# DoHoonKim8/stark-verifier

Measured on AMD Instinct MI355X. Metric: recursive plonky2 proofs/sec (Semaphore d=20), higher is better.
Workload: dtype u64 (Goldilocks field, integer); 1 GPU; recursive: per unit one Semaphore signal (group 2^20, n=2^13, blowup 8, 28 FRI queries, 16 PoW bits, zk) + the recursive proof verifying it (n=2^14, same FRI parameters); 128 units per GPU per step, 10 prover contexts per GPU; all_gather of (nullifier|topic) + Poseidon aggregation root per step; parallelism=independent proofs sharded over ranks, no data-path collective, exchange=none (one rank): gl355_aggregation_root over the local leaves, units_proven_in_process=1674

## Files before the change

include/gl355.h:

```cpp
#ifndef GL355_H
#define GL355_H
#include <stddef.h>
#include <stdint.h>

#ifdef __cplusplus
extern "C" {
#endif

#define GL355_OK 0
#define GL355_E_INVALID_ARG (-1)
#define GL355_E_NO_DEVICE (-2)
#define GL355_E_OOM (-3)
#define GL355_E_HIP (-4)
#define GL355_E_UNSUPPORTED (-5)
#define GL355_E_WITNESS (-6)
#define GL355_E_VERIFY (-7)

#define GL355_P UINT64_C(0xFFFFFFFF00000001)
#define GL355_COSET_SHIFT UINT64_C(7)
#define GL355_SALT_SIZE 4
#define GL355_MAX_UNITS 16

typedef struct gl355_ctx gl355_ctx;
typedef struct gl355_oracle gl355_oracle;
// ... 122 lines not shown
int32_t gl355_quotient_values(gl355_ctx* ctx, const gl355_circuit* circuit, const gl355_oracle* constants_sigmas,
                              const gl355_oracle* wires, const gl355_oracle* zs_partial_products, const uint64_t* k_is,
                              const uint64_t* betas, const uint64_t* gammas, const uint64_t* alphas,
                              const uint64_t pi_hash[4], uint64_t* values);

typedef struct { const gl355_oracle* oracle; uint32_t column; } gl355_poly_ref;
int32_t gl355_deep_batch(gl355_ctx* ctx, const gl355_poly_ref* polys, uint32_t n_polys,
                         const uint64_t alpha[2], const uint64_t z[2], uint64_t* acc);
int32_t gl355_eval_polys(gl355_ctx* ctx, const gl355_poly_ref* polys, uint32_t n_polys,
                         const uint64_t z[2], uint64_t* out);
int32_t gl355_lde_ext(gl355_ctx* ctx, const uint64_t* coeffs, uint32_t log_n, uint32_t rate_bits,
                      uint64_t shift, uint64_t* out);

int32_t gl355_fri_fold(gl355_ctx* ctx, const uint64_t* coeffs, uint64_t n, const uint64_t beta[2], uint64_t* out);
int32_t gl355_fri_layer_commit_h(gl355_ctx* ctx, int32_t hasher, const uint64_t* values, uint64_t n, uint32_t cap_height,
                                 uint64_t* leaves, uint64_t* digests, uint64_t* cap);
int32_t gl355_fri_layer_commit(gl355_ctx* ctx, const uint64_t* values, uint64_t n, uint32_t cap_height,
                               uint64_t* leaves, uint64_t* digests, uint64_t* cap);

int32_t gl355_pow_grind_h(gl355_ctx* ctx, int32_t hasher, const uint64_t state[12], uint32_t pos, uint32_t bits, uint64_t start,
                          uint64_t* witness);
int32_t gl355_pow_grind(gl355_ctx* ctx, const uint64_t state[12], uint32_t pos, uint32_t bits,
                        uint64_t start, uint64_t* witness);

typedef struct {
    uint64_t state[12];
    uint64_t in_buf[8];
    uint32_t in_len;
    uint64_t out_buf[8];
    uint32_t out_len;
    int32_t hasher;
} gl355_challenger;
int32_t gl355_challenger_init(gl355_challenger* c);
int32_t gl355_challenger_init_h(gl355_challenger* c, int32_t hasher);
int32_t gl355_challenger_observe(gl355_challenger* c, const uint64_t* elems, uint64_t n);
int32_t gl355_challenger_squeeze(gl355_challenger* c, uint64_t* out, uint64_t n);
int32_t gl355_challenger_pow_state(const gl355_challenger* c, uint64_t state[12], uint32_t* pos);
int32_t gl355_host_poseidon_permute(uint64_t state[12]);
int32_t gl355_host_hash_no_pad(const uint64_t* in, uint64_t len, uint64_t out[4]);
int32_t gl355_host_permute_h(int32_t hasher, uint64_t state[12]);
int32_t gl355_host_hash_no_pad_h(int32_t hasher, const uint64_t* in, uint64_t len, uint64_t out[4]);
int32_t gl355_poseidon_gate_witness(const uint64_t inputs[12], uint64_t swap, uint64_t wires[135]);

int32_t gl355_fri_prove(gl355_ctx* ctx, const uint64_t* final_coeffs, uint32_t log_n, uint32_t rate_bits,
                        uint32_t cap_height, const uint32_t* arity_bits, uint32_t n_layers, uint32_t pow_bits,
                        uint32_t num_queries, gl355_challenger* ch, uint64_t* caps, uint64_t* final_poly,
// ... 166 lines not shown
```

stark-verifier_amd/_lib.py:

```python
import ctypes as C
import os

_HERE = os.path.dirname(os.path.abspath(__file__))
LIB_PATH = os.path.join(_HERE, "lib", "libgl355.so")

u64p = C.POINTER(C.c_uint64)
vp = C.c_void_p


class Gl355Error(RuntimeError):
    def __init__(self, code, msg):
        super().__init__("gl355 error %d: %s" % (code, msg))
        self.code = code


class PolyRef(C.Structure):
    _fields_ = [("oracle", vp), ("column", C.c_uint32)]


class Challenger(C.Structure):
    _fields_ = [("state", C.c_uint64 * 12), ("in_buf", C.c_uint64 * 8), ("in_len", C.c_uint32),
                ("out_buf", C.c_uint64 * 8), ("out_len", C.c_uint32), ("hasher", C.c_int32)]


# ... 123 lines not shown
    "gl355_witness_replay_segmented": (C.c_int32, [vp, C.c_uint64, C.c_uint64, vp, C.c_uint32, C.c_uint32, vp, C.c_uint64, vp, C.c_uint64, C.c_uint32,
                                                   C.POINTER(C.c_uint64)]),
    "gl355_witness_replay": (C.c_int32, [vp, C.c_uint64, vp, C.c_uint64, vp, C.c_uint64, C.c_uint32, C.POINTER(C.c_uint64)]),
    "gl355_quotient": (C.c_int32, [vp, C.POINTER(Circuit), vp, vp, vp, vp, vp, vp, vp, vp, vp]),
    "gl355_quotient_values": (C.c_int32, [vp, C.POINTER(Circuit), vp, vp, vp, vp, vp, vp, vp, vp, vp]),
    "gl355_challenger_init": (C.c_int32, [C.POINTER(Challenger)]),
    "gl355_challenger_init_h": (C.c_int32, [C.POINTER(Challenger), C.c_int32]),
    "gl355_challenger_observe": (C.c_int32, [C.POINTER(Challenger), vp, C.c_uint64]),
    "gl355_challenger_squeeze": (C.c_int32, [C.POINTER(Challenger), vp, C.c_uint64]),
    "gl355_challenger_pow_state": (C.c_int32, [C.POINTER(Challenger), vp, C.POINTER(C.c_uint32)]),
    "gl355_host_poseidon_permute": (C.c_int32, [vp]),
    "gl355_host_hash_no_pad": (C.c_int32, [vp, C.c_uint64, vp]),
    "gl355_host_hash_no_pad_h": (C.c_int32, [C.c_int32, vp, C.c_uint64, vp]),
    "gl355_host_permute_h": (C.c_int32, [C.c_int32, vp]),
    "gl355_poseidon_gate_witness": (C.c_int32, [vp, C.c_uint64, vp]),
    "gl355_deep_batch": (C.c_int32, [vp, C.POINTER(PolyRef), C.c_uint32, vp, vp, vp]),
    "gl355_eval_polys": (C.c_int32, [vp, C.POINTER(PolyRef), C.c_uint32, vp, vp]),
    "gl355_lde_ext": (C.c_int32, [vp, vp, C.c_uint32, C.c_uint32, C.c_uint64, vp]),
    "gl355_fri_fold": (C.c_int32, [vp, vp, C.c_uint64, vp, vp]),
    "gl355_fri_layer_commit_h": (C.c_int32, [vp, C.c_int32, vp, C.c_uint64, C.c_uint32, vp, vp, vp]),
    "gl355_fri_layer_commit": (C.c_int32, [vp, vp, C.c_uint64, C.c_uint32, vp, vp, vp]),
    "gl355_pow_grind_h": (C.c_int32, [vp, C.c_int32, vp, C.c_uint32, C.c_uint32, C.c_uint64, C.POINTER(C.c_uint64)]),
    "gl355_pow_grind": (C.c_int32, [vp, vp, C.c_uint32, C.c_uint32, C.c_uint64, C.POINTER(C.c_uint64)]),
    "gl355_comm_unique_id": (C.c_int32, [C.c_int32, C.c_char_p]),
    "gl355_comm_host_id": (C.c_int32, [C.c_char_p, C.c_uint16, C.c_char_p]),
    "gl355_comm_create": (C.c_int32, [vp, C.c_int32, C.c_char_p, C.c_int32, C.c_int32, C.POINTER(vp)]),
    "gl355_comm_destroy": (C.c_int32, [vp]),
    "gl355_comm_info": (C.c_int32, [vp, C.POINTER(C.c_int32), C.POINTER(C.c_int32), C.POINTER(C.c_int32)]),
    "gl355_comm_last_error": (C.c_char_p, [vp]),
    "gl355_gather_digests": (C.c_int32, [vp, vp, C.c_uint64, vp]),
    "gl355_comm_barrier": (C.c_int32, [vp]),
    "gl355_comm_max_f64": (C.c_int32, [vp, C.POINTER(C.c_double)]),
    "gl355_aggregation_root": (C.c_int32, [vp, vp, C.c_uint64, C.c_uint32, vp]),
    "gl355_bn254_fr_ntt": (C.c_int32, [vp, vp, C.c_uint32, C.c_int32]),
    "gl355_bn254_fr_coset_ntt": (C.c_int32, [vp, vp, C.c_uint32, C.c_uint32, vp, C.c_int32, vp]),
    "gl355_bn254_g1_msm": (C.c_int32, [vp, vp, vp, C.c_uint64, vp]),
    "gl355_bn254_g1_msm_batch": (C.c_int32, [vp, vp, vp, C.c_uint64, C.c_uint32, vp]),
    "gl355_bn254_g1_msm_prepare": (C.c_int32, [vp, vp, C.c_uint64, C.POINTER(vp)]),
    "gl355_bn254_g1_msm_prepared": (C.c_int32, [vp, vp, vp, C.c_uint32, vp]),
    "gl355_bn254_g1_msm_bases_free": (C.c_int32, [vp, vp]),
    "gl355_bn254_g1_fixed_base_mul": (C.c_int32, [vp, vp, vp, C.c_uint64, vp]),
    "gl355_bn254_g1_fft": (C.c_int32, [vp, vp, C.c_uint32, C.c_int32]),
    "gl355_kzg_setup": (C.c_int32, [vp, vp, C.c_uint32, vp, vp]),
    "gl355_kzg_lagrange_from_powers": (C.c_int32, [vp, vp, C.c_uint64, C.c_uint32, vp]),
    "gl355_kzg_commit": (C.c_int32, [vp, vp, vp, C.c_uint32, C.c_int32, vp]),
    "gl355_kzg_open": (C.c_int32, [vp, vp, vp, C.c_uint32, vp, vp, vp, vp]),
# ... 32 lines not shown
```

stark-verifier_amd/api.py:

```python
import ctypes as C

import numpy as np

from . import _lib
from ._lib import Gl355Error, PolyRef

P = (1 << 64) - (1 << 32) + 1
COSET_SHIFT = 7
SALT_SIZE = 4


def _ptr(x):
    if x is None:
        return None
    if isinstance(x, np.ndarray):
        assert x.dtype == np.uint64 and x.flags["C_CONTIGUOUS"], "need C-contiguous uint64"
        return x.ctypes.data_as(C.c_void_p)
    if isinstance(x, int):
        return C.c_void_p(x)
    if hasattr(x, "data_ptr"):
        assert x.is_contiguous()
        return C.c_void_p(x.data_ptr())
    raise TypeError("unsupported buffer type %r" % type(x))

# ... 144 lines not shown

    def fri_fold(self, coeffs_ext, beta):
        c = _u64(coeffs_ext)
        n = c.size // 2
        out = np.empty(n, dtype=np.uint64)
        b = _u64(beta)
        self.check(self.lib.gl355_fri_fold(self.h, _ptr(c), n, _ptr(b), _ptr(out)))
        return out

    def fri_layer_commit(self, values_ext, cap_height):
        v = _u64(values_ext)
        n = v.size // 2
        leaves = np.empty((n // 2, 4), dtype=np.uint64)
        digests = np.empty((2 * (n // 2 - (1 << cap_height)), 4), dtype=np.uint64)
        cap = np.empty((1 << cap_height, 4), dtype=np.uint64)
        self.check(self.lib.gl355_fri_layer_commit(self.h, _ptr(v), n, cap_height, _ptr(leaves), _ptr(digests), _ptr(cap)))
        return MerkleTree._from_parts(self, leaves, digests, cap, cap_height)

    def pow_grind(self, state, pos, bits, start=0):
        s = _u64(state)
        w = C.c_uint64()
        self.check(self.lib.gl355_pow_grind(self.h, _ptr(s), pos, bits, start, C.byref(w)))
        return w.value

    def zs_partial_products(self, wires, sigmas, k_is, max_degree, beta, gamma):
        w, s, k = _u64(wires), _u64(sigmas), _u64(k_is)
        n_routed, n = w.shape
        n_chunks = (n_routed + max_degree - 1) // max_degree
        z = np.empty(n, dtype=np.uint64)
        pp = np.empty((n_chunks - 1, n), dtype=np.uint64)
        self.check(self.lib.gl355_zs_partial_products(self.h, _ptr(w), _ptr(s), _ptr(k), int(n).bit_length() - 1,
                                                      n_routed, max_degree, beta, gamma, _ptr(z), _ptr(pp)))
        return z, pp


class _Hasher:
    ID = HASH_POSEIDON

    def __init__(self, ctx):
        self.ctx = ctx

    def permute(self, states):
        st = _u64(states).copy()
        s2 = st.reshape(-1, 12)
        self.ctx.check(self.ctx.lib.gl355_permute_h(self.ctx.h, self.ID, _ptr(s2), s2.shape[0]))
        return st
# ... 191 lines not shown
```

stark-verifier_amd/csrc/capi.hip:

```cpp
#include "gl355_internal.h"

using namespace gl355;

namespace gl355 {

int32_t ntt_dev(Ctx* ctx, uint64_t* data, uint32_t log_n, uint32_t batch, uint64_t stride, bool inverse,
                uint64_t coset_shift) {
    if (batch == 0) return GL355_OK;
    const uint64_t n = 1ull << log_n;
    if (log_n > 24) return ctx->fail(GL355_E_UNSUPPORTED, "ntt: log_n > 24 unsupported");
    NttPlan p;
    p.in = data; p.out = data; p.in_col_stride = stride; p.out_col_stride = stride;
    p.log_n = log_n; p.batch = batch; p.inverse = inverse;
    const bool coset = coset_shift != 0 && gl_canon(coset_shift) != 1;
    if (!inverse) {
        if (coset) GL355_TRY(ctx->pow_tables(coset_shift, &p.pre_lo, &p.pre_hi));
        p.out_bitrev = false;
        return ntt_run(ctx, p);
    }
    p.scale = gl_canon(gl_inv(n % GL_P));
    if (log_n <= 14) {
        if (coset) GL355_TRY(ctx->pow_tables(gl_inv(coset_shift), &p.post_lo, &p.post_hi));
        return ntt_run(ctx, p);
    }
// ... 503 lines not shown
    if (cap_height > lg) return ctx->fail(GL355_E_INVALID_ARG, "fri_layer_commit: cap_height too large");
    const uint64_t n_cap = 1ull << cap_height, n_dig = 2 * (n_leaves - n_cap);
    Staged sv(ctx), sl(ctx), sd(ctx), sc(ctx);
    GL355_TRY(sv.open(values, n * 16, 1));
    GL355_TRY(sl.open(leaves, n * 16, 2));
    GL355_TRY(sd.open(digests, n_dig * 32, 2));
    GL355_TRY(sc.open(cap, n_cap * 32, 2));
    GL355_TRY(fri_layer_leaves_dev(ctx, sv.as<uint64_t>(), n, sl.as<uint64_t>()));
    GL355_TRY(merkle_build_any(ctx, hasher, sl.as<uint64_t>(), n_leaves, 4, false, 0, cap_height, sd.as<uint64_t>(), sc.as<uint64_t>()));
    GL355_TRY(sl.finish());
    GL355_TRY(sd.finish());
    return sc.finish();
}
int32_t gl355_pow_grind(gl355_ctx* h, const uint64_t state[12], uint32_t pos, uint32_t bits, uint64_t start, uint64_t* witness) {
    return gl355_pow_grind_h(h, GL355_HASH_POSEIDON, state, pos, bits, start, witness);
}
int32_t gl355_pow_grind_h(gl355_ctx* h, int32_t hasher, const uint64_t state[12], uint32_t pos, uint32_t bits, uint64_t start,
                          uint64_t* witness) {
    CTX_OR_FAIL(h);
    HASHER_OR_FAIL(hasher);
    if (!state || !witness || pos >= 8) return ctx->fail(GL355_E_INVALID_ARG, "pow_grind: bad argument");
    return pow_grind_any(ctx, hasher, state, pos, bits, start, witness);
}

int32_t gl355_zs_partial_products(gl355_ctx* h, const uint64_t* wires, const uint64_t* sigmas, const uint64_t* k_is,
                                  uint32_t log_n, uint32_t n_routed, uint32_t max_degree, uint64_t beta, uint64_t gamma,
                                  uint64_t* z_out, uint64_t* pp_out) {
    CTX_OR_FAIL(h);
    if (n_routed == 0 || max_degree == 0 || log_n > 24) return ctx->fail(GL355_E_INVALID_ARG, "zs_partial_products: bad shape");
    const uint64_t n = 1ull << log_n;
    const uint32_t n_chunks = (n_routed + max_degree - 1) / max_degree;
    Staged sw(ctx), ss(ctx), sk(ctx), sz(ctx), sp(ctx);
    GL355_TRY(sw.open(wires, (uint64_t)n_routed * n * 8, 1));
    GL355_TRY(ss.open(sigmas, (uint64_t)n_routed * n * 8, 1));
    GL355_TRY(sk.open(k_is, (uint64_t)n_routed * 8, 1));
    GL355_TRY(sz.open(z_out, n * 8, 2));
    GL355_TRY(sp.open(pp_out, (uint64_t)(n_chunks - 1) * n * 8, 2));
    GL355_TRY(zs_partial_products_dev(ctx, sw.as<uint64_t>(), ss.as<uint64_t>(), sk.as<uint64_t>(), log_n, n_routed, max_degree,
                                      beta, gamma, sz.as<uint64_t>(), sp.as<uint64_t>()));
    GL355_TRY(sz.finish());
    return sp.finish();
}

}
```

stark-verifier_amd/csrc/gl355_internal.h:

```cpp
#pragma once
#include <hip/hip_runtime.h>
#include <stdint.h>
#include <string.h>

#include <algorithm>
#include <map>
#include <mutex>
#include <string>
#include <vector>

#include "../../include/gl355.h"
#include "gl_field.cuh"
#include "merkle_common.cuh"

namespace gl355 { struct Ctx; }

struct gl355_oracle {
    struct gl355::Ctx* ctx;
    uint32_t log_n, rate_bits, batch, leaf_len, cap_height;
    uint64_t* coeffs;
    uint64_t* lde;
    uint64_t* digests;
    uint64_t* cap;
    uint64_t n_digests;
// ... 164 lines not shown
int32_t two_to_one_dev(Ctx* ctx, const uint64_t* l, const uint64_t* r, uint64_t n, uint64_t* out);
int32_t open_batch_dev(Ctx* ctx, const uint64_t* lde, uint64_t stride, uint32_t leaf_len, const uint64_t* digests,
                       uint32_t log_n, uint32_t cap_height, const uint64_t* idx_dev, uint32_t n_idx, uint64_t* leaves_out,
                       uint64_t* sib_out);
int32_t open_batch_ex_dev(Ctx* ctx, const uint64_t* leaves, uint64_t stride, uint32_t leaf_len, const uint64_t* digests,
                          uint32_t log_n, uint32_t cap_height, const uint64_t* idx_dev, uint32_t idx_shift, uint32_t n_idx,
                          uint64_t* leaves_out, uint64_t leaf_out_stride, uint64_t* sib_out, uint64_t sib_out_stride);
void host_bn254_permute(uint64_t state[12]);
int32_t merkle_build_any(Ctx* ctx, int32_t hasher, const uint64_t* leaves, uint64_t n_leaves, uint32_t leaf_len, bool col_major,
                         uint64_t col_stride, uint32_t cap_height, uint64_t* digests, uint64_t* cap);
int32_t pow_grind_any(Ctx* ctx, int32_t hasher, const uint64_t state[12], uint32_t pos, uint32_t bits, uint64_t start,
                      uint64_t* witness_host);
int32_t bn254_pow_grind_dev(Ctx* ctx, const uint64_t state[12], uint32_t pos, uint32_t bits, uint64_t start, uint64_t* witness_host);
int32_t bn254_permute_dev(Ctx* ctx, uint64_t* states, uint64_t count);
int32_t bn254_hash_leaves_dev(Ctx* ctx, const uint64_t* leaves, uint64_t n_leaves, uint32_t leaf_len, bool col_major, uint64_t col_stride,
                              uint64_t* digests, bool always_hash);
int32_t bn254_two_to_one_dev(Ctx* ctx, const uint64_t* l, const uint64_t* r, uint64_t n, uint64_t* out);
int32_t bn254_merkle_build_dev(Ctx* ctx, const uint64_t* leaves, uint64_t n_leaves, uint32_t leaf_len, bool col_major, uint64_t col_stride,
                               uint32_t cap_height, uint64_t* digests, uint64_t* cap);
int32_t oracle_open_batch_on(Ctx* ctx, const gl355_oracle* o, const uint64_t* indices, uint32_t n_idx, uint64_t* leaves,
                             uint64_t* siblings);
int32_t pow_grind_dev(Ctx* ctx, const uint64_t state[12], uint32_t pos, uint32_t bits, uint64_t start,
                      uint64_t* witness_host);

int32_t deep_batch_dev(Ctx* ctx, const uint64_t* const* poly_ptrs_host, uint32_t n_polys, uint32_t log_n,
                       const uint64_t alpha[2], const uint64_t z[2], uint64_t* acc );
int32_t eval_polys_ext_dev(Ctx* ctx, const uint64_t* const* poly_ptrs_host, uint32_t n_polys, uint32_t log_n,
                           const uint64_t z[2], uint64_t* out_host_or_dev);
int32_t fri_fold_dev(Ctx* ctx, const uint64_t* coeffs, uint64_t n, const uint64_t beta[2], uint64_t* out);
int32_t fri_layer_leaves_dev(Ctx* ctx, const uint64_t* values, uint64_t n, uint64_t* leaves);
int32_t lde_ext_dev(Ctx* ctx, const uint64_t* coeffs, uint32_t log_n, uint32_t rate_bits, uint64_t shift, uint64_t* out,
                    bool out_bitrev);
int32_t field_batch_dev(Ctx* ctx, int32_t op, const uint64_t* a, const uint64_t* b, uint64_t* out, uint64_t n);
int32_t zs_partial_products_dev(Ctx* ctx, const uint64_t* wires, const uint64_t* sigmas, const uint64_t* k_is,
                                uint32_t log_n, uint32_t n_routed, uint32_t max_degree, uint64_t beta, uint64_t gamma,
                                uint64_t* z_out, uint64_t* pp_out);
int32_t canon_dev(Ctx* ctx, uint64_t* a, uint64_t n);
int32_t intt_from_bitrev_dev(Ctx* ctx, const uint64_t* in, uint64_t in_stride, uint64_t* out, uint64_t out_stride,
                             uint32_t log_n, uint32_t batch, uint64_t coset_shift);
int32_t quotient_dev(Ctx* ctx, const gl355_circuit* c, const uint64_t* cs_lde, const uint64_t* wires_lde,
                     const uint64_t* zs_lde, uint64_t lde_stride, const uint64_t* k_is_dev, const uint64_t* betas,
                     const uint64_t* gammas, const uint64_t* alphas, const uint64_t pi_hash[4], uint64_t* out_values);
Ctx* ctx_of(gl355_ctx* h);
uint64_t thread_cpu_ns();

struct BlindKey;
// ... 32 lines not shown
```

stark-verifier_amd/csrc/merkle.hip:

```cpp
#include "gl355_internal.h"
#include "poseidon.cuh"
#include "merkle_common.cuh"

namespace gl355 {


__global__ void __launch_bounds__(256) poseidon_permute_kernel(uint64_t* states, uint64_t count) {
    const uint64_t i = blockIdx.x * (uint64_t)blockDim.x + threadIdx.x;
    if (i >= count) return;
    uint64_t s[12];
#pragma unroll
    for (int k = 0; k < 12; k++) s[k] = states[i * 12 + k];
    psd_permute(s);
#pragma unroll
    for (int k = 0; k < 12; k++) states[i * 12 + k] = gl_canon(s[k]);
}


#ifndef PSD_LEAF_WAVES
#define PSD_LEAF_WAVES 4
#endif
__global__ void __launch_bounds__(256) __attribute__((amdgpu_waves_per_eu(PSD_LEAF_WAVES))) hash_leaves_kernel(LeafArgs a) {
    const uint64_t i = blockIdx.x * (uint64_t)blockDim.x + threadIdx.x;
    if (i >= a.n_leaves) return;
// ... 170 lines not shown
                if (valid && li < 4) {
                    const uint64_t v = gl_canon(s);
                    lvl[cur ^ 1][j * 4 + li] = v;
                    uint64_t* dst = (layer == sub_bits) ? cap + t * 4 : tree + digest_slot(layer, (uint64_t)j) * 4;
                    dst[li] = v;
                }
            }
        }
        __syncthreads();
        cur ^= 1;
    }
}

__global__ void __launch_bounds__(256) two_to_one_kernel(const uint64_t* l, const uint64_t* r, uint64_t n, uint64_t* out) {
    const uint64_t i = blockIdx.x * (uint64_t)blockDim.x + threadIdx.x;
    if (i >= n) return;
    uint64_t s[12] = {l[4 * i], l[4 * i + 1], l[4 * i + 2], l[4 * i + 3],
                      r[4 * i], r[4 * i + 1], r[4 * i + 2], r[4 * i + 3], 0, 0, 0, 0};
    psd_permute(s);
#pragma unroll
    for (int k = 0; k < 4; k++) out[4 * i + k] = gl_canon(s[k]);
}

__global__ void __launch_bounds__(256) pow_grind_kernel(const uint64_t* state, uint32_t pos, uint32_t bits,
                                                       uint64_t start, unsigned long long* best) {
    const uint64_t w = start + blockIdx.x * (uint64_t)blockDim.x + threadIdx.x;
    if (w > __hip_atomic_load(best, __ATOMIC_RELAXED, __HIP_MEMORY_SCOPE_AGENT)) return;
    uint64_t s[12];
#pragma unroll
    for (int k = 0; k < 12; k++) s[k] = state[k];
#pragma unroll
    for (int k = 0; k < 12; k++) if ((uint32_t)k == pos) s[k] = w;
    psd_permute(s);
    const uint64_t resp = gl_canon(s[7]);
    if (bits == 0 || (resp >> (64 - bits)) == 0) atomicMin(best, (unsigned long long)w);
}

__global__ void open_batch_kernel(const uint64_t* lde, uint64_t stride, uint32_t leaf_len, const uint64_t* digests,
                                  uint32_t log_n, uint32_t cap_height, const uint64_t* idx, uint32_t idx_shift,
                                  uint64_t* leaves_out, uint64_t leaf_out_stride, uint64_t* sib_out, uint64_t sib_out_stride) {
    const uint64_t index = idx[blockIdx.x] >> idx_shift;
    const uint32_t layers = log_n - cap_height;
    for (uint32_t c = threadIdx.x; c < leaf_len; c += blockDim.x)
        leaves_out[(uint64_t)blockIdx.x * leaf_out_stride + c] = stride ? lde[(uint64_t)c * stride + index] : lde[index * leaf_len + c];
    const uint64_t sub_leaves = 1ull << layers;
    const uint64_t* tree = digests + (index >> layers) * 2 * (sub_leaves - 1) * 4;
    const uint64_t k0 = index & (sub_leaves - 1);
    for (uint32_t e = threadIdx.x; e < layers * 4; e += blockDim.x) {
        const uint32_t layer = e >> 2;
        const uint64_t k = (k0 >> layer) ^ 1;
        sib_out[(uint64_t)blockIdx.x * sib_out_stride + layer * 4 + (e & 3)] = tree[digest_slot(layer, k) * 4 + (e & 3)];
    }
}

int32_t open_batch_dev(Ctx* ctx, const uint64_t* lde, uint64_t stride, uint32_t leaf_len, const uint64_t* digests,
                       uint32_t log_n, uint32_t cap_height, const uint64_t* idx_dev, uint32_t n_idx, uint64_t* leaves_out,
                       uint64_t* sib_out) {
    if (n_idx == 0) return GL355_OK;
// ... 81 lines not shown
        const uint64_t n_nodes = n_leaves >> layer;
        if (layer == top_from) {
            ProfScope ps(ctx, "merkle_top_kernel", (2 * n_nodes - (n_leaves >> sub_bits)) * 96);
            if (fast_lanes) hipLaunchKernelGGL(merkle_top_kernel<3>, dim3((uint32_t)(n_leaves >> sub_bits)), dim3(1024), 0, ctx->stream, digests, cap, sub_bits, layer, top_levels);
            else hipLaunchKernelGGL(merkle_top_kernel<0>, dim3((uint32_t)(n_leaves >> sub_bits)), dim3(1024), 0, ctx->stream, digests, cap, sub_bits, layer, top_levels);
            GL355_HIP(ctx, hipGetLastError());
            break;
        }
        ProfScope ps(ctx, n_nodes <= lanes_max ? "merkle_level_lanes_kernel" : "merkle_level_kernel", n_nodes * 96);
        if (n_nodes <= lanes_max) {
            if (fast_lanes) hipLaunchKernelGGL(merkle_level_lanes_kernel<3>, dim3((uint32_t)((n_nodes + 3) / 4)), dim3(64), 0, ctx->stream,
                                               digests, cap, sub_bits, layer, n_nodes);
            else hipLaunchKernelGGL(merkle_level_lanes_kernel<0>, dim3((uint32_t)((n_nodes + 3) / 4)), dim3(64), 0, ctx->stream,
                                    digests, cap, sub_bits, layer, n_nodes);
        } else {
            hipLaunchKernelGGL(merkle_level_kernel, dim3((uint32_t)((n_nodes + 255) / 256)), dim3(256), 0, ctx->stream,
                               digests, cap, sub_bits, layer, n_nodes);
        }
        GL355_HIP(ctx, hipGetLastError());
    }
    return GL355_OK;
}

int32_t pow_grind_dev(Ctx* ctx, const uint64_t state[12], uint32_t pos, uint32_t bits, uint64_t start,
                      uint64_t* witness_host) {
    if (pos >= 8) return ctx->fail(GL355_E_INVALID_ARG, "pow: witness position must be in the rate part");
    if (bits > 40) return ctx->fail(GL355_E_UNSUPPORTED, "pow: more than 40 bits of grinding refused");
    Scratch sc(ctx);
    GL355_TRY(sc.get(13 * sizeof(uint64_t)));
    uint64_t* d_state = sc.as<uint64_t>();
    unsigned long long* d_best = reinterpret_cast<unsigned long long*>(d_state + 12);
    uint64_t host[13];
    for (int i = 0; i < 12; i++) host[i] = gl_canon(state[i]);
    host[12] = ~0ull;
    GL355_HIP(ctx, hipMemcpyAsync(d_state, host, sizeof host, hipMemcpyHostToDevice, ctx->stream));
    uint64_t per_launch = 1ull << std::min<uint32_t>(std::max<uint32_t>(bits + 1, 12), 22);
    uint64_t base = start;
    for (;;) {
        ProfScope ps(ctx, "pow_grind", 0);
        hipLaunchKernelGGL(pow_grind_kernel, dim3((uint32_t)(per_launch / 256)), dim3(256), 0, ctx->stream, d_state, pos,
                           bits, base, d_best);
        GL355_HIP(ctx, hipGetLastError());
        unsigned long long best;
        GL355_HIP(ctx, ctx->d2h(&best, d_best, sizeof best));
        GL355_HIP(ctx, ctx->wait());
        if (best != ~0ull) { *witness_host = best; return GL355_OK; }
        base += per_launch;
        if (per_launch < (1ull << 22)) per_launch <<= 1;
        if (base - start > (1ull << 44)) return ctx->fail(GL355_E_UNSUPPORTED, "pow: no witness found in 2^44 candidates");
    }
}

}
```

stark-verifier_amd/csrc/poseidon.cuh:

```cuda
#pragma once
#include "gl_field.cuh"

#define PSD_TABLE_QUAL __device__ __constant__ const
#include "poseidon_tables.h"

namespace gl355 {

#ifndef PSD_SBOX_INTERLEAVE
#define PSD_SBOX_INTERLEAVE 1
#endif
#ifndef PSD_SBOX_WIDTH
#define PSD_SBOX_WIDTH 4
#endif
GL_DEV uint64_t psd_sbox(uint64_t x) {
#if PSD_SBOX_INTERLEAVE && defined(__HIP_DEVICE_COMPILE__) && GL_MUL_VARIANT == 1
    const uint64_t x2 = gl_sqr(x);
    const uint64_t a[2] = {x, x2}, b[2] = {x2, x2};
    uint64_t r[2];
    gl_mul_multi<2>(a, b, r);
    return gl_mul(r[0], r[1]);
#else
    uint64_t x2 = gl_sqr(x), x4 = gl_sqr(x2), x3 = gl_mul(x, x2);
    return gl_mul(x3, x4);
#endif
// ... 271 lines not shown
                for (int i = 0; i < 12; i += 4) psd_sbox4(s[i], s[i + 1], s[i + 2], s[i + 3]);
#else
                for (int i = 0; i < 12; i += 2) psd_sbox2(s[i], s[i + 1]);
#endif
            } else {
                s[0] = psd_sbox(s[0]);
            }
            psd_mds(s, &PSD_ALL_RC[12 * (r + h + 1)]);
        }
    }
}
GL_DEV void psd_permute(uint64_t (&s)[12]) {
#pragma unroll
    for (int i = 0; i < 12; i++) s[i] = gl_add_canonical(s[i], PSD_ALL_RC[i]);
    psd_dense_rounds<true>(s, 0, 4);
#if PSD_PARTIAL_FORM == 1
    psd_partial_rounds_block(s);
#else
    psd_dense_rounds<false>(s, 4, 26);
#endif
    psd_dense_rounds<true>(s, 26, 30);
}

struct PsdSponge {
    uint64_t s[12];
    GL_DEV void init() {
#pragma unroll
        for (int i = 0; i < 12; i++) s[i] = 0;
    }
};

}
```

stark-verifier_amd/csrc/prover_batch.hip:

```cpp
#include "gl355_internal.h"
#include "blinding.cuh"
#include "poseidon.cuh"

using namespace gl355;

namespace gl355 {

constexpr uint32_t MAXB = GL355_MAX_UNITS;

struct BOracle {
    Ctx* ctx = nullptr;
    uint32_t B = 0, log_n = 0, rate_bits = 0, batch = 0, leaf_len = 0, cap_height = 0;
    uint64_t* base = nullptr;
    uint64_t *coeffs = nullptr, *lde = nullptr, *salt = nullptr, *digests = nullptr, *cap = nullptr;
    uint64_t n_dig = 0;
    ~BOracle() { if (base && ctx) ctx->release(base); }
    int32_t alloc(Ctx* c, uint32_t b, uint32_t lg, uint32_t rb, uint32_t bat, bool salted, uint32_t cap_h) {
        ctx = c; B = b; log_n = lg; rate_bits = rb; batch = bat; leaf_len = bat + (salted ? GL355_SALT_SIZE : 0); cap_height = cap_h;
        const uint64_t n = 1ull << lg, N = n << rb, n_cap = 1ull << cap_h;
        n_dig = 2 * (N - n_cap);
        const uint64_t total = (uint64_t)B * ((uint64_t)bat * n + (uint64_t)leaf_len * N + n_dig * 4 + n_cap * 4);
        void* p = nullptr;
        GL355_TRY(c->alloc(total * 8, &p));
        base = reinterpret_cast<uint64_t*>(p);
// ... 303 lines not shown
    if (i >= len / 2) return;
    const uint32_t u = blockIdx.y;
    const uint64_t* c0 = cols + (uint64_t)u * 2 * len;
    const uint64_t* c1 = c0 + len;
    const ulonglong2 a = *reinterpret_cast<const ulonglong2*>(c0 + 2 * i);
    const ulonglong2 b = *reinterpret_cast<const ulonglong2*>(c1 + 2 * i);
    uint64_t* dst = leaves + ((uint64_t)u * (len / 2) + i) * 4;
    *reinterpret_cast<ulonglong2*>(dst) = make_ulonglong2(a.x, b.x);
    *reinterpret_cast<ulonglong2*>(dst + 2) = make_ulonglong2(a.y, b.y);
}
__global__ void fri_fold_units_kernel(const uint64_t* cols , uint64_t len, UnitVals beta, uint64_t* out ) {
    const uint64_t k = blockIdx.x * (uint64_t)blockDim.x + threadIdx.x;
    const uint64_t half = len / 2;
    if (k >= half) return;
    const uint32_t u = blockIdx.y;
    const uint64_t* c0 = cols + (uint64_t)u * 2 * len;
    const uint64_t* c1 = c0 + len;
    const ulonglong2 a = *reinterpret_cast<const ulonglong2*>(c0 + 2 * k);
    const ulonglong2 b = *reinterpret_cast<const ulonglong2*>(c1 + 2 * k);
    const gl2 r = gl2_canon(gl2_add(gl2_make(a.x, b.x), gl2_mul(gl2_make(a.y, b.y), gl2_make(beta.v[u * 4], beta.v[u * 4 + 1]))));
    uint64_t* o0 = out + (uint64_t)u * 2 * half;
    o0[k] = r.c0; o0[half + k] = r.c1;
}
struct PowArgs { uint64_t state[MAXB * 12]; uint32_t pos[MAXB]; uint32_t todo[MAXB]; uint32_t bits; uint64_t start; unsigned long long* best; };
__global__ void __launch_bounds__(256) pow_grind_units_kernel(PowArgs a) {
    const uint32_t u = blockIdx.y;
    if (!a.todo[u]) return;
    const uint64_t w = a.start + blockIdx.x * (uint64_t)blockDim.x + threadIdx.x;
    if (w > __hip_atomic_load(a.best + u, __ATOMIC_RELAXED, __HIP_MEMORY_SCOPE_AGENT)) return;
    uint64_t s[12];
#pragma unroll
    for (int k = 0; k < 12; k++) s[k] = a.state[u * 12 + k];
#pragma unroll
    for (int k = 0; k < 12; k++) if ((uint32_t)k == a.pos[u]) s[k] = w;
    psd_permute(s);
    const uint64_t resp = gl_canon(s[7]);
    if (a.bits == 0 || (resp >> (64 - a.bits)) == 0) atomicMin(a.best + u, (unsigned long long)w);
}

struct OpenArgs { OView o; uint64_t N; uint32_t lde_bits, cap_height, n_idx; const uint64_t* idx ; uint64_t* leaves; uint64_t* sibs; };
__global__ void open_units_kernel(OpenArgs a) {
    const uint32_t q = blockIdx.x, u = blockIdx.y;
    const uint64_t index = a.idx[(uint64_t)u * a.n_idx + q];
    const uint32_t layers = a.lde_bits - a.cap_height;
    const uint64_t* lde = a.o.lde + (uint64_t)u * a.o.lde_us;
    const uint64_t* salt = a.o.salt ? a.o.salt + (uint64_t)u * a.o.salt_us : nullptr;
    uint64_t* lo = a.leaves + ((uint64_t)u * a.n_idx + q) * a.o.leaf_len;
    for (uint32_t c = threadIdx.x; c < a.o.leaf_len; c += blockDim.x)
        lo[c] = c < a.o.batch ? lde[(uint64_t)c * a.N + index] : salt[(uint64_t)(c - a.o.batch) * a.N + index];
    const uint64_t sub_leaves = 1ull << layers;
    const uint64_t* tree = a.o.digests + (uint64_t)u * a.o.dig_us + (index >> layers) * 2 * (sub_leaves - 1) * 4;
    const uint64_t k0 = index & (sub_leaves - 1);
    uint64_t* so = a.sibs + ((uint64_t)u * a.n_idx + q) * layers * 4;
    for (uint32_t e = threadIdx.x; e < layers * 4; e += blockDim.x) {
        const uint32_t layer = e >> 2;
        const uint64_t k = (k0 >> layer) ^ 1;
        so[e] = tree[digest_slot(layer, k) * 4 + (e & 3)];
    }
}
struct OpenFriArgs {
    const uint64_t* trees; uint64_t leaf_off[32], dig_off[32];
    uint64_t sib_off[32], sib_total;
// ... 291 lines not shown
        GL355_TRY(merkle_build_args_any(ctx, hasher, la, log2_u64(nl) - cap_h, tree_buf + dig_off[l], d_cap));
        GL355_HIP(ctx, ctx->d2h(stage, d_cap, (uint64_t)B * n_cap * 32));
        GL355_HIP(ctx, ctx->wait());
        UnitVals beta;
        memset(&beta, 0, sizeof beta);
        for (uint32_t u = 0; u < B; u++) {
            uint64_t* dst = p_fri_caps[u] + (uint64_t)l * n_cap * 4;
            memcpy(dst, stage + (uint64_t)u * n_cap * 4, n_cap * 32);
            gl355_challenger_observe(&ch[u], dst, n_cap * 4);
            gl355_challenger_squeeze(&ch[u], &beta.v[u * 4], 2);
            beta.v[u * 4] = gl_canon(beta.v[u * 4]); beta.v[u * 4 + 1] = gl_canon(beta.v[u * 4 + 1]);
        }
        {
            ProfScope ps(ctx, "fri_fold", (uint64_t)B * (len_c * 16 + len_c * 8));
            hipLaunchKernelGGL(fri_fold_units_kernel, dim3((uint32_t)((len_c / 2 + 255) / 256), B), dim3(256), 0, ctx->stream, cols, len_c, beta, cols2);
            LAUNCH_CHECK(ctx);
        }
        std::swap(cols, cols2);
        len_c >>= 1;
        shift = gl_mul(shift, shift);
    }
    GL355_HIP(ctx, ctx->d2h(stage, cols, (uint64_t)B * 2 * len_c * 8));
    GL355_HIP(ctx, ctx->wait());
    PowArgs pa;
    memset(&pa, 0, sizeof pa);
    std::vector<uint64_t*> p_pow(B);
    for (uint32_t u = 0; u < B; u++) {
        const uint64_t* c0 = stage + (uint64_t)u * 2 * len_c;
        for (uint64_t k = 0; k < len_c; k++) { out[u][2 * k] = c0[k]; out[u][2 * k + 1] = c0[len_c + k]; }
        gl355_challenger_observe(&ch[u], out[u], 2 * len_c);
        out[u] += 2 * len_c;
        p_pow[u] = out[u]; out[u] += 1;
        uint64_t st[12];
        uint32_t pos;
        if (gl355_challenger_pow_state(&ch[u], st, &pos) != GL355_OK) return ctx->fail(GL355_E_INVALID_ARG, "prove: challenger state");
        for (int k = 0; k < 12; k++) pa.state[u * 12 + k] = gl_canon(st[k]);
        pa.pos[u] = pos; pa.todo[u] = 1;
    }
    if (hasher == GL355_HASH_POSEIDON) {
        if (pd->pow_bits > 40) return ctx->fail(GL355_E_UNSUPPORTED, "pow: more than 40 bits of grinding refused");
        Scratch pb(ctx);
        GL355_TRY(pb.get(MAXB * 8));
        pa.best = reinterpret_cast<unsigned long long*>(pb.p);
        pa.bits = pd->pow_bits;
        GL355_HIP(ctx, hipMemsetAsync(pb.p, 0xFF, MAXB * 8, ctx->stream));
        uint64_t per_launch = 1ull << std::min<uint32_t>(std::max<uint32_t>(pd->pow_bits + 1, 12), 22);
        uint64_t base = 0;
        for (uint32_t left = B; left;) {
            ProfScope ps(ctx, "pow_grind", 0);
            pa.start = base;
            hipLaunchKernelGGL(pow_grind_units_kernel, dim3((uint32_t)(per_launch / 256), B), dim3(256), 0, ctx->stream, pa);
            LAUNCH_CHECK(ctx);
            GL355_HIP(ctx, ctx->d2h(stage, pb.p, (uint64_t)B * 8));
            GL355_HIP(ctx, ctx->wait());
            for (uint32_t u = 0; u < B; u++)
                if (pa.todo[u] && stage[u] != ~0ull) { *p_pow[u] = stage[u]; pa.todo[u] = 0; left--; }
            base += per_launch;
            if (per_launch < (1ull << 22)) per_launch <<= 1;
            if (base > (1ull << 44)) return ctx->fail(GL355_E_UNSUPPORTED, "pow: no witness found in 2^44 candidates");
        }
    } else {
        for (uint32_t u = 0; u < B; u++) GL355_TRY(pow_grind_any(ctx, hasher, &pa.state[u * 12], pa.pos[u], pd->pow_bits, 0, p_pow[u]));
    }
    std::vector<uint64_t> q_idx((uint64_t)B * nq_idx);
    for (uint32_t u = 0; u < B; u++) {
        gl355_challenger_observe(&ch[u], p_pow[u], 1);
        uint64_t resp;
        gl355_challenger_squeeze(&ch[u], &resp, 1);
        if (pd->pow_bits && (resp >> (64 - pd->pow_bits)) != 0) return ctx->fail(GL355_E_HIP, "prove: proof-of-work response check failed");
        gl355_challenger_squeeze(&ch[u], &q_idx[(uint64_t)u * nq_idx], nq_idx);
        for (uint32_t q = 0; q < nq_idx; q++) q_idx[(uint64_t)u * nq_idx + q] &= (N - 1);
    }
    Scratch ob(ctx);
    GL355_TRY(ob.get(((uint64_t)B * nq_idx + (uint64_t)B * open_words + 16) * 8));
    uint64_t* d_idx = ob.as<uint64_t>();
    uint64_t* d_open = d_idx + (uint64_t)B * nq_idx;
    GL355_HIP(ctx, hipMemcpyAsync(d_idx, q_idx.data(), (uint64_t)B * nq_idx * 8, hipMemcpyHostToDevice, ctx->stream));
    uint64_t off_leaf[4], off_sib[4], woff = 0;
    for (int o = 0; o < 4; o++) {
        off_leaf[o] = woff; woff += (uint64_t)B * nq_idx * leaf_lens[o];
        off_sib[o] = woff; woff += (uint64_t)B * nq_idx * depth0 * 4;
        OpenArgs oa;
        oa.o = *vs[o]; oa.N = N; oa.lde_bits = lde_bits; oa.cap_height = cap_h; oa.n_idx = nq_idx; oa.idx = d_idx;
        oa.leaves = d_open + off_leaf[o]; oa.sibs = d_open + off_sib[o];
        if (oa.o.leaf_len != leaf_lens[o]) return ctx->fail(GL355_E_HIP, "prove: internal leaf-length mismatch");
// ... 44 lines not shown
```

Baseline: 317.1 recursive proofs/s.

## Grind PoW in one persistent kernel with precomputed first round

```diff
diff --git a/include/gl355.h b/include/gl355.h
--- a/include/gl355.h
+++ b/include/gl355.h
@@ -168,6 +168,8 @@
                           uint64_t* witness);
 int32_t gl355_pow_grind(gl355_ctx* ctx, const uint64_t state[12], uint32_t pos, uint32_t bits,
                         uint64_t start, uint64_t* witness);
+int32_t gl355_pow_grind_units(gl355_ctx* ctx, uint32_t n_units, const uint64_t* states, const uint32_t* pos, uint32_t bits, uint64_t start,
+                              uint64_t* witness);
 
 typedef struct {
     uint64_t state[12];
diff --git a/stark-verifier_amd/_lib.py b/stark-verifier_amd/_lib.py
--- a/stark-verifier_amd/_lib.py
+++ b/stark-verifier_amd/_lib.py
@@ -169,6 +169,7 @@
     "gl355_fri_layer_commit": (C.c_int32, [vp, vp, C.c_uint64, C.c_uint32, vp, vp, vp]),
     "gl355_pow_grind_h": (C.c_int32, [vp, C.c_int32, vp, C.c_uint32, C.c_uint32, C.c_uint64, C.POINTER(C.c_uint64)]),
     "gl355_pow_grind": (C.c_int32, [vp, vp, C.c_uint32, C.c_uint32, C.c_uint64, C.POINTER(C.c_uint64)]),
+    "gl355_pow_grind_units": (C.c_int32, [vp, C.c_uint32, vp, vp, C.c_uint32, C.c_uint64, vp]),
     "gl355_comm_unique_id": (C.c_int32, [C.c_int32, C.c_char_p]),
     "gl355_comm_host_id": (C.c_int32, [C.c_char_p, C.c_uint16, C.c_char_p]),
     "gl355_comm_create": (C.c_int32, [vp, C.c_int32, C.c_char_p, C.c_int32, C.c_int32, C.POINTER(vp)]),
diff --git a/stark-verifier_amd/api.py b/stark-verifier_amd/api.py
--- a/stark-verifier_amd/api.py
+++ b/stark-verifier_amd/api.py
@@ -190,6 +190,14 @@
         w = C.c_uint64()
         self.check(self.lib.gl355_pow_grind(self.h, _ptr(s), pos, bits, start, C.byref(w)))
         return w.value
+
+    def pow_grind_units(self, states, pos, bits, start=0):
+        s = _u64(states).reshape(-1, 12)
+        p = np.ascontiguousarray(pos, dtype=np.uint32)
+        assert p.shape == (s.shape[0],)
+        w = np.empty(s.shape[0], dtype=np.uint64)
+        self.check(self.lib.gl355_pow_grind_units(self.h, s.shape[0], _ptr(s), p.ctypes.data_as(C.c_void_p), bits, start, _ptr(w)))
+        return w
 
     def zs_partial_products(self, wires, sigmas, k_is, max_degree, beta, gamma):
         w, s, k = _u64(wires), _u64(sigmas), _u64(k_is)
diff --git a/stark-verifier_amd/csrc/capi.hip b/stark-verifier_amd/csrc/capi.hip
--- a/stark-verifier_amd/csrc/capi.hip
+++ b/stark-verifier_amd/csrc/capi.hip
@@ -549,6 +549,12 @@
     if (!state || !witness || pos >= 8) return ctx->fail(GL355_E_INVALID_ARG, "pow_grind: bad argument");
     return pow_grind_any(ctx, hasher, state, pos, bits, start, witness);
 }
+int32_t gl355_pow_grind_units(gl355_ctx* h, uint32_t n_units, const uint64_t* states, const uint32_t* pos, uint32_t bits, uint64_t start,
+                              uint64_t* witness) {
+    CTX_OR_FAIL(h);
+    if (!states || !pos || !witness || n_units == 0 || n_units > GL355_MAX_UNITS) return ctx->fail(GL355_E_INVALID_ARG, "pow_grind_units: bad argument");
+    return pow_grind_units_dev(ctx, n_units, states, pos, bits, start, witness);
+}
 
 int32_t gl355_zs_partial_products(gl355_ctx* h, const uint64_t* wires, const uint64_t* sigmas, const uint64_t* k_is,
                                   uint32_t log_n, uint32_t n_routed, uint32_t max_degree, uint64_t beta, uint64_t gamma,
diff --git a/stark-verifier_amd/csrc/gl355_internal.h b/stark-verifier_amd/csrc/gl355_internal.h
--- a/stark-verifier_amd/csrc/gl355_internal.h
+++ b/stark-verifier_amd/csrc/gl355_internal.h
@@ -210,6 +210,8 @@
                              uint64_t* siblings);
 int32_t pow_grind_dev(Ctx* ctx, const uint64_t state[12], uint32_t pos, uint32_t bits, uint64_t start,
                       uint64_t* witness_host);
+int32_t pow_grind_units_dev(Ctx* ctx, uint32_t n, const uint64_t* states, const uint32_t* pos, uint32_t bits, uint64_t start,
+                            uint64_t* witnesses);
 
 int32_t deep_batch_dev(Ctx* ctx, const uint64_t* const* poly_ptrs_host, uint32_t n_polys, uint32_t log_n,
                        const uint64_t alpha[2], const uint64_t z[2], uint64_t* acc );
diff --git a/stark-verifier_amd/csrc/merkle.hip b/stark-verifier_amd/csrc/merkle.hip
--- a/stark-verifier_amd/csrc/merkle.hip
+++ b/stark-verifier_amd/csrc/merkle.hip
@@ -216,18 +216,37 @@
     for (int k = 0; k < 4; k++) out[4 * i + k] = gl_canon(s[k]);
 }
 
-__global__ void __launch_bounds__(256) pow_grind_kernel(const uint64_t* state, uint32_t pos, uint32_t bits,
-                                                       uint64_t start, unsigned long long* best) {
-    const uint64_t w = start + blockIdx.x * (uint64_t)blockDim.x + threadIdx.x;
-    if (w > __hip_atomic_load(best, __ATOMIC_RELAXED, __HIP_MEMORY_SCOPE_AGENT)) return;
-    uint64_t s[12];
-#pragma unroll
-    for (int k = 0; k < 12; k++) s[k] = state[k];
-#pragma unroll
-    for (int k = 0; k < 12; k++) if ((uint32_t)k == pos) s[k] = w;
-    psd_permute(s);
-    const uint64_t resp = gl_canon(s[7]);
-    if (bits == 0 || (resp >> (64 - bits)) == 0) atomicMin(best, (unsigned long long)w);
+struct PowStates { uint64_t state[GL355_MAX_UNITS * 12]; uint32_t pos[GL355_MAX_UNITS]; };
+__global__ void pow_pre_kernel(PowStates in, uint32_t n, PsdPowPre* pre) {
+    const uint32_t u = threadIdx.x;
+    if (u >= n) return;
+    uint64_t st[12];
+#pragma unroll
+    for (int k = 0; k < 12; k++) st[k] = in.state[u * 12 + k];
+    psd_pow_pre(st, in.pos[u], pre[u]);
+}
+constexpr uint64_t POW_GIVE_UP = 1ull << 44;
+#ifndef POW_UNIT_SHARE_LOG
+#define POW_UNIT_SHARE_LOG 4
+#endif
+__global__ void __launch_bounds__(256) pow_grind_kernel(const PsdPowPre* __restrict__ pre, uint32_t n, uint32_t bits, uint64_t start,
+                                                       unsigned long long* best, unsigned long long* next) {
+    const uint32_t lane = threadIdx.x & 63;
+    const uint32_t u = __builtin_amdgcn_readfirstlane((blockIdx.x * (blockDim.x >> 6) + (threadIdx.x >> 6)) % n);
+    uint64_t k[12];
+    uint32_t col[12];
+#pragma unroll
+    for (int r = 0; r < 12; r++) { k[r] = pre[u].k[r]; col[r] = pre[u].col[r]; }
+    const uint64_t rc_pos = pre[u].rc_pos;
+    for (;;) {
+        unsigned long long c = 0;
+        if (lane == 0) c = atomicAdd(next + u, 64ull);
+        c = ((uint64_t)__builtin_amdgcn_readfirstlane((uint32_t)(c >> 32)) << 32) | __builtin_amdgcn_readfirstlane((uint32_t)c);
+        if (c >= POW_GIVE_UP || start + c > __hip_atomic_load(best + u, __ATOMIC_RELAXED, __HIP_MEMORY_SCOPE_AGENT)) break;
+        const uint64_t w = start + c + lane;
+        const uint64_t resp = gl_canon(psd_pow_lane7(k, col, rc_pos, w));
+        if (bits == 0 || (resp >> (64 - bits)) == 0) atomicMin(best + u, (unsigned long long)w);
+    }
 }
 
 __global__ void open_batch_kernel(const uint64_t* lde, uint64_t stride, uint32_t leaf_len, const uint64_t* digests,
@@ -355,33 +374,52 @@
     return GL355_OK;
 }
 
+int32_t pow_grind_units_dev(Ctx* ctx, uint32_t n, const uint64_t* states, const uint32_t* pos, uint32_t bits, uint64_t start,
+                            uint64_t* witnesses) {
+    if (n == 0 || n > GL355_MAX_UNITS) return ctx->fail(GL355_E_INVALID_ARG, "pow: bad number of proofs");
+    if (bits > 40) return ctx->fail(GL355_E_UNSUPPORTED, "pow: more than 40 bits of grinding refused");
+    if (start > ~0ull - POW_GIVE_UP) return ctx->fail(GL355_E_INVALID_ARG, "pow: start too large");
+    PowStates in;
+    memset(&in, 0, sizeof in);
+    for (uint32_t u = 0; u < n; u++) {
+        if (pos[u] >= 8) return ctx->fail(GL355_E_INVALID_ARG, "pow: witness position must be in the rate part");
+        for (int i = 0; i < 12; i++) in.state[u * 12 + i] = gl_canon(states[u * 12 + i]);
+        in.pos[u] = pos[u];
+    }
+    int per_cu = 0, n_cu = 0;
+    GL355_HIP(ctx, hipOccupancyMaxActiveBlocksPerMultiprocessor(&per_cu, pow_grind_kernel, 256, 0));
+    GL355_HIP(ctx, hipDeviceGetAttribute(&n_cu, hipDeviceAttributeMultiprocessorCount, ctx->device));
+    if (per_cu < 1 || n_cu < 1) return ctx->fail(GL355_E_HIP, "pow: no occupancy");
+    const uint64_t lone = 1ull << std::min<uint32_t>(std::max<uint32_t>(bits + 1, 12), 22);
+    const uint64_t want = std::max<uint64_t>(lone, (uint64_t)n * (lone >> POW_UNIT_SHARE_LOG)) / 256;
+    const uint32_t blocks = (uint32_t)std::max<uint64_t>(n, std::min<uint64_t>(want, (uint64_t)per_cu * n_cu));
+    Scratch sc(ctx);
+    GL355_TRY(sc.get(n * sizeof(PsdPowPre) + 2 * GL355_MAX_UNITS * sizeof(uint64_t)));
+    PsdPowPre* d_pre = sc.as<PsdPowPre>();
+    unsigned long long* d_best = reinterpret_cast<unsigned long long*>(d_pre + n);
+    unsigned long long* d_next = d_best + GL355_MAX_UNITS;
+    GL355_HIP(ctx, hipMemsetAsync(d_best, 0xFF, GL355_MAX_UNITS * sizeof(uint64_t), ctx->stream));
+    GL355_HIP(ctx, hipMemsetAsync(d_next, 0, GL355_MAX_UNITS * sizeof(uint64_t), ctx->stream));
+    {
+        ProfScope ps(ctx, "pow_grind", 0);
+        hipLaunchKernelGGL(pow_pre_kernel, dim3(1), dim3(64), 0, ctx->stream, in, n, d_pre);
+        hipLaunchKernelGGL(pow_grind_kernel, dim3(blocks), dim3(256), 0, ctx->stream, d_pre, n, bits, start, d_best, d_next);
+        GL355_HIP(ctx, hipGetLastError());
+    }
+    uint64_t best[GL355_MAX_UNITS];
+    GL355_HIP(ctx, ctx->d2h(best, d_best, n * sizeof(uint64_t)));
+    GL355_HIP(ctx, ctx->wait());
+    for (uint32_t u = 0; u < n; u++) {
+        if (best[u] == ~0ull) return ctx->fail(GL355_E_UNSUPPORTED, "pow: no witness found in 2^44 candidates");
+        witnesses[u] = best[u];
+    }
+    return GL355_OK;
+}
+
 int32_t pow_grind_dev(Ctx* ctx, const uint64_t state[12], uint32_t pos, uint32_t bits, uint64_t start,
                       uint64_t* witness_host) {
     if (pos >= 8) return ctx->fail(GL355_E_INVALID_ARG, "pow: witness position must be in the rate part");
-    if (bits > 40) return ctx->fail(GL355_E_UNSUPPORTED, "pow: more than 40 bits of grinding refused");
-    Scratch sc(ctx);
-    GL355_TRY(sc.get(13 * sizeof(uint64_t)));
-    uint64_t* d_state = sc.as<uint64_t>();
-    unsigned long long* d_best = reinterpret_cast<unsigned long long*>(d_state + 12);
-    uint64_t host[13];
-    for (int i = 0; i < 12; i++) host[i] = gl_canon(state[i]);
-    host[12] = ~0ull;
-    GL355_HIP(ctx, hipMemcpyAsync(d_state, host, sizeof host, hipMemcpyHostToDevice, ctx->stream));
-    uint64_t per_launch = 1ull << std::min<uint32_t>(std::max<uint32_t>(bits + 1, 12), 22);
-    uint64_t base = start;
-    for (;;) {
-        ProfScope ps(ctx, "pow_grind", 0);
-        hipLaunchKernelGGL(pow_grind_kernel, dim3((uint32_t)(per_launch / 256)), dim3(256), 0, ctx->stream, d_state, pos,
-                           bits, base, d_best);
-        GL355_HIP(ctx, hipGetLastError());
-        unsigned long long best;
-        GL355_HIP(ctx, ctx->d2h(&best, d_best, sizeof best));
-        GL355_HIP(ctx, ctx->wait());
-        if (best != ~0ull) { *witness_host = best; return GL355_OK; }
-        base += per_launch;
-        if (per_launch < (1ull << 22)) per_launch <<= 1;
-        if (base - start > (1ull << 44)) return ctx->fail(GL355_E_UNSUPPORTED, "pow: no witness found in 2^44 candidates");
-    }
-}
-
-}
+    return pow_grind_units_dev(ctx, 1, state, &pos, bits, start, witness_host);
+}
+
+}
diff --git a/stark-verifier_amd/csrc/poseidon.cuh b/stark-verifier_amd/csrc/poseidon.cuh
--- a/stark-verifier_amd/csrc/poseidon.cuh
+++ b/stark-verifier_amd/csrc/poseidon.cuh
@@ -317,6 +317,58 @@
     psd_dense_rounds<true>(s, 26, 30);
 }
 
+struct PsdPowPre {
+    uint64_t k[12];
+    uint64_t rc_pos;
+    uint32_t col[12];
+};
+GL_HD uint32_t psd_mds_entry(int r, int c) {
+    constexpr uint32_t circ[12] = {17, 15, 41, 16, 2, 28, 13, 13, 39, 18, 34, 20};
+    return circ[(c - r + 12) % 12] + (r == 0 && c == 0 ? 8u : 0u);
+}
+GL_DEV void psd_pow_pre(const uint64_t (&st)[12], uint32_t pos, PsdPowPre& pre) {
+    uint64_t t[12];
+#pragma unroll
+    for (int c = 0; c < 12; c++) t[c] = (uint32_t)c == pos ? 0 : psd_sbox(gl_add_canonical(st[c], PSD_ALL_RC[c]));
+#pragma unroll
+    for (int r = 0; r < 12; r++) {
+        uint64_t acc = PSD_ALL_RC[12 + r];
+#pragma unroll
+        for (int c = 0; c < 12; c++) acc = gl_add(acc, gl_mul_small(t[c], psd_mds_entry(r, c)));
+        pre.k[r] = gl_canon(acc);
+        pre.col[r] = psd_mds_entry(r, (int)pos);
+    }
+    pre.rc_pos = PSD_ALL_RC[pos];
+}
+GL_DEV void psd_full_round(uint64_t (&s)[12], int r) {
+#pragma unroll
+    for (int i = 0; i < 12; i += 4) psd_sbox4(s[i], s[i + 1], s[i + 2], s[i + 3]);
+    psd_mds(s, &PSD_ALL_RC[12 * (r + 1)]);
+}
+GL_DEV uint64_t psd_pow_lane7(const uint64_t (&k)[12], const uint32_t (&col)[12], uint64_t rc_pos, uint64_t w) {
+    const uint64_t x = psd_sbox(gl_add_canonical(w, rc_pos));
+    const uint32_t xl = (uint32_t)x, xh = (uint32_t)(x >> 32);
+    uint64_t s[12];
+#pragma unroll
+    for (int r = 0; r < 12; r++)
+        s[r] = psd_recombine((uint64_t)col[r] * xl + (uint32_t)k[r], (uint64_t)col[r] * xh + (k[r] >> 32));
+    psd_dense_rounds<true>(s, 1, 3);
+    psd_full_round(s, 3);
+#if PSD_PARTIAL_FORM == 1
+    psd_partial_rounds_block(s);
+#else
+    psd_dense_rounds<false>(s, 4, 26);
+#endif
+    psd_dense_rounds<true>(s, 26, 28);
+    psd_full_round(s, 28);
+#pragma unroll
+    for (int i = 0; i < 12; i += 4) psd_sbox4(s[i], s[i + 1], s[i + 2], s[i + 3]);
+    uint32_t lo[12], hi[12];
+#pragma unroll
+    for (int i = 0; i < 12; i++) { lo[i] = (uint32_t)s[i]; hi[i] = (uint32_t)(s[i] >> 32); }
+    return psd_recombine(psd_mds_chain<7>(lo, 0), psd_mds_chain<7>(hi, 0));
+}
+
 struct PsdSponge {
     uint64_t s[12];
     GL_DEV void init() {
diff --git a/stark-verifier_amd/csrc/prover_batch.hip b/stark-verifier_amd/csrc/prover_batch.hip
--- a/stark-verifier_amd/csrc/prover_batch.hip
+++ b/stark-verifier_amd/csrc/prover_batch.hip
@@ -349,22 +349,6 @@
     uint64_t* o0 = out + (uint64_t)u * 2 * half;
     o0[k] = r.c0; o0[half + k] = r.c1;
 }
-struct PowArgs { uint64_t state[MAXB * 12]; uint32_t pos[MAXB]; uint32_t todo[MAXB]; uint32_t bits; uint64_t start; unsigned long long* best; };
-__global__ void __launch_bounds__(256) pow_grind_units_kernel(PowArgs a) {
-    const uint32_t u = blockIdx.y;
-    if (!a.todo[u]) return;
-    const uint64_t w = a.start + blockIdx.x * (uint64_t)blockDim.x + threadIdx.x;
-    if (w > __hip_atomic_load(a.best + u, __ATOMIC_RELAXED, __HIP_MEMORY_SCOPE_AGENT)) return;
-    uint64_t s[12];
-#pragma unroll
-    for (int k = 0; k < 12; k++) s[k] = a.state[u * 12 + k];
-#pragma unroll
-    for (int k = 0; k < 12; k++) if ((uint32_t)k == a.pos[u]) s[k] = w;
-    psd_permute(s);
-    const uint64_t resp = gl_canon(s[7]);
-    if (a.bits == 0 || (resp >> (64 - a.bits)) == 0) atomicMin(a.best + u, (unsigned long long)w);
-}
-
 struct OpenArgs { OView o; uint64_t N; uint32_t lde_bits, cap_height, n_idx; const uint64_t* idx ; uint64_t* leaves; uint64_t* sibs; };
 __global__ void open_units_kernel(OpenArgs a) {
     const uint32_t q = blockIdx.x, u = blockIdx.y;
@@ -702,8 +686,8 @@
     }
     GL355_HIP(ctx, ctx->d2h(stage, cols, (uint64_t)B * 2 * len_c * 8));
     GL355_HIP(ctx, ctx->wait());
-    PowArgs pa;
-    memset(&pa, 0, sizeof pa);
+    std::vector<uint64_t> pow_state((uint64_t)B * 12);
+    std::vector<uint32_t> pow_pos(B);
     std::vector<uint64_t*> p_pow(B);
     for (uint32_t u = 0; u < B; u++) {
         const uint64_t* c0 = stage + (uint64_t)u * 2 * len_c;
@@ -711,36 +695,16 @@
         gl355_challenger_observe(&ch[u], out[u], 2 * len_c);
         out[u] += 2 * len_c;
         p_pow[u] = out[u]; out[u] += 1;
-        uint64_t st[12];
-        uint32_t pos;
-        if (gl355_challenger_pow_state(&ch[u], st, &pos) != GL355_OK) return ctx->fail(GL355_E_INVALID_ARG, "prove: challenger state");
-        for (int k = 0; k < 12; k++) pa.state[u * 12 + k] = gl_canon(st[k]);
-        pa.pos[u] = pos; pa.todo[u] = 1;
+        if (gl355_challenger_pow_state(&ch[u], &pow_state[(uint64_t)u * 12], &pow_pos[u]) != GL355_OK)
+            return ctx->fail(GL355_E_INVALID_ARG, "prove: challenger state");
+        for (int k = 0; k < 12; k++) pow_state[(uint64_t)u * 12 + k] = gl_canon(pow_state[(uint64_t)u * 12 + k]);
     }
     if (hasher == GL355_HASH_POSEIDON) {
-        if (pd->pow_bits > 40) return ctx->fail(GL355_E_UNSUPPORTED, "pow: more than 40 bits of grinding refused");
-        Scratch pb(ctx);
-        GL355_TRY(pb.get(MAXB * 8));
-        pa.best = reinterpret_cast<unsigned long long*>(pb.p);
-        pa.bits = pd->pow_bits;
-        GL355_HIP(ctx, hipMemsetAsync(pb.p, 0xFF, MAXB * 8, ctx->stream));
-        uint64_t per_launch = 1ull << std::min<uint32_t>(std::max<uint32_t>(pd->pow_bits + 1, 12), 22);
-        uint64_t base = 0;
-        for (uint32_t left = B; left;) {
-            ProfScope ps(ctx, "pow_grind", 0);
-            pa.start = base;
-            hipLaunchKernelGGL(pow_grind_units_kernel, dim3((uint32_t)(per_launch / 256), B), dim3(256), 0, ctx->stream, pa);
-            LAUNCH_CHECK(ctx);
-            GL355_HIP(ctx, ctx->d2h(stage, pb.p, (uint64_t)B * 8));
-            GL355_HIP(ctx, ctx->wait());
-            for (uint32_t u = 0; u < B; u++)
-                if (pa.todo[u] && stage[u] != ~0ull) { *p_pow[u] = stage[u]; pa.todo[u] = 0; left--; }
-            base += per_launch;
-            if (per_launch < (1ull << 22)) per_launch <<= 1;
-            if (base > (1ull << 44)) return ctx->fail(GL355_E_UNSUPPORTED, "pow: no witness found in 2^44 candidates");
-        }
+        std::vector<uint64_t> w(B);
+        GL355_TRY(pow_grind_units_dev(ctx, B, pow_state.data(), pow_pos.data(), pd->pow_bits, 0, w.data()));
+        for (uint32_t u = 0; u < B; u++) *p_pow[u] = w[u];
     } else {
-        for (uint32_t u = 0; u < B; u++) GL355_TRY(pow_grind_any(ctx, hasher, &pa.state[u * 12], pa.pos[u], pd->pow_bits, 0, p_pow[u]));
+        for (uint32_t u = 0; u < B; u++) GL355_TRY(pow_grind_any(ctx, hasher, &pow_state[(uint64_t)u * 12], pow_pos[u], pd->pow_bits, 0, p_pow[u]));
     }
     std::vector<uint64_t> q_idx((uint64_t)B * nq_idx);
     for (uint32_t u = 0; u < B; u++) {
```

Result: no change. 317.2 recursive proofs/s (median of 6 runs) (+0.0%).
